# vitskvara/VBMatrixFactorization.jl

Measured on NVIDIA B200. Metric: VB iterations/s at 20000x200000x64 (dense vbmf, Float64), higher is better.
Workload: dtype f64

## Files before the change

### vbmatrixfactorization.jl_b200/csrc/capi.cu

```cuda
#include "../../include/vbmf_b200.h"
#include "common.cuh"
#include "gemm.cuh"
#include "kernels.cuh"

#include <atomic>
#include <type_traits>
#include <cstdarg>
#include <cstdlib>
#include <cstring>
#include <dlfcn.h>
#include <unistd.h>
#include <string>
#include <vector>
#include <algorithm>
#include <thread>

namespace vb {

static thread_local char g_err[1024] = "";
void set_error(const char* fmt, ...) {
    va_list ap;
    va_start(ap, fmt);
    vsnprintf(g_err, sizeof(g_err), fmt, ap);
    va_end(ap);
// ... 46 lines not shown
        }                                                                                       \
    } while (0)

}

using namespace vb;

struct vbmf_b200_ctx {
    int device = 0, rank = 0, world = 1, num_sms = 148;
    cudaStream_t st = nullptr;
    bool own_stream = false;
    void* comm = nullptr;
    double* Y = nullptr;
    size_t Y_cap = 0;
    int L_cap = 0;
    int L = 0, Mloc = 0, Mglob = 0, moff = 0, ldY = 0;
    double* rowY2 = nullptr;
    double* d_tr = nullptr;
    double* stats_part = nullptr;
    double trYTY = 0.0;
    CUtensorMap tmY1, tmY2;
    bool have_Y = false;
    cudaStream_t copy_st = nullptr, stat_st = nullptr;
    std::vector<cudaEvent_t> ev_chunk;
    std::vector<int> chunk_c0, chunk_n;
    cudaEvent_t ev_stats = nullptr;
    int chunks_pending = 0;
    bool tr_pending = false;
    bool simt = false;
    bool gemm_dmma = false;
    uint8_t* Z = nullptr;
    int* Zexp = nullptr;
    size_t Z_bytes = 0;
    int ldZ = 0;
    bool z_ready = false, z_failed = false;
    CUtensorMap tmZ1, tmZ2;
    bool profile = false;
    std::vector<cudaEvent_t> ev_k1, ev_k2, ev_ar;
    std::vector<std::pair<int, cudaEvent_t>> ev_seg;
    struct Px {
        bool ok = false, failed = false, claimed = false;
        char* local = nullptr;
        size_t cap = 0;
        char* peer[PX_MAX_WORLD] = {};
        bool ipc[PX_MAX_WORLD] = {};
        char* xchg = nullptr;
        unsigned long long epoch = 0;
        unsigned long long* wait_ns = nullptr;
    } px;
    bool profile_segments = false;
    char* batch_dev = nullptr;
    char* batch_host = nullptr;
    size_t batch_bytes = 0;
};

static int ctx_allreduce(vbmf_b200_ctx* c, double* buf, size_t n) {
    if (c->world <= 1 || n == 0) return 0;
    VB_NCCL_OK(g_nccl.AllReduce(buf, buf, n,  8,  0, c->comm, c->st));
    return 0;
}

struct PxRec {
    long long pid;
    unsigned long long host;
    unsigned long long ptr;
    int dev, ok;
    cudaIpcMemHandle_t h;
    char pad[128 - 32 - sizeof(cudaIpcMemHandle_t)];
};
// ... 279 lines not shown
        if (ctx_allreduce(c, c->rowY2, (size_t)c->L)) return -1;
        if (k_total(c->st, c->rowY2, c->L, c->d_tr)) return -1;
    }
    VB_CUDA_OK(cudaMemcpyAsync(&c->trYTY, c->d_tr, 8, cudaMemcpyDeviceToHost, c->st));
    VB_CUDA_OK(cudaStreamSynchronize(c->st));
    c->have_Y = true;
    return 0;
}

static int ctx_wait_upload(vbmf_b200_ctx* c) {
    if (c->chunks_pending > 0) {
        VB_CUDA_OK(cudaStreamWaitEvent(c->st, c->ev_stats, 0));
        c->chunks_pending = 0;
    }
    return 0;
}
static int ctx_host_trYTY(vbmf_b200_ctx* c) {
    if (c->tr_pending) {
        VB_CUDA_OK(cudaEventSynchronize(c->ev_stats));
        VB_CUDA_OK(cudaMemcpy(&c->trYTY, c->d_tr, 8, cudaMemcpyDeviceToHost));
        c->tr_pending = false;
    }
    return 0;
}
static size_t align_up(size_t x, size_t a) { return (x + a - 1) / a * a; }

static bool ctx_int8_wanted(const vbmf_b200_ctx* c, int64_t H) {
    return !c->simt && !c->gemm_dmma && H >= 1 && H <= 64 && c->Y != nullptr && c->Mloc > 0;
}
static int ctx_slices(vbmf_b200_ctx* c, bool* ok) {
    *ok = false;
    if (c->z_failed || c->Y == nullptr || c->Mloc <= 0) return 0;
    if (c->z_ready) { *ok = true; return 0; }
    const int ldZ = i8_ld(c->L);
    const size_t bytes = (size_t)I8_NSL * c->Mloc * ldZ;
    if (c->Z == nullptr || c->Z_bytes != bytes || c->ldZ != ldZ) {
        ctx_free_Z(c);
        if (cudaMalloc(&c->Z, bytes) != cudaSuccess || cudaMalloc(&c->Zexp, 2 * ((size_t)ldZ + c->Mloc) * 4) != cudaSuccess) {
            cudaGetLastError();
            ctx_free_Z(c);
            c->z_failed = true;
            return 0;
        }
        c->Z_bytes = bytes; c->ldZ = ldZ;
    }
    int* F = c->Zexp;
    if (i8_build_Y(c->st, c->Y, c->ldY, c->L, c->Mloc, c->Z, ldZ, F, F + c->L, F + c->L + c->Mloc, F + 2 * c->L + c->Mloc)) return -1;
    const uint64_t s1 = (uint64_t)ldZ, s2 = (uint64_t)ldZ * c->Mloc;
    if (make_tmap_3d_i8(&c->tmZ1, c->Z, (uint64_t)c->L, (uint64_t)c->Mloc, I8_NSL, s1, s2, 32, 128, I8_NSL, false)) return -1;
    if (make_tmap_3d_i8(&c->tmZ2, c->Z, (uint64_t)c->L, (uint64_t)c->Mloc, I8_NSL, s1, s2, 128, 32, I8_NSL, true)) return -1;
    c->z_ready = true;
    *ok = true;
    return 0;
}
static void i8_plans(int L, int M, int H, int num_sms, int* S1, int* kbs1, int* S, int* kchunk) {
    plan_splitk_ytb(L, M, H, num_sms, S1, kbs1);
    *kbs1 = (*kbs1 + 1) & ~1;
    const int nkb = (L + 15) / 16;
    *S1 = std::max(1, (nkb + *kbs1 - 1) / *kbs1);
    plan_splitk(L, M, H, num_sms, S, kchunk);
    *kchunk = (*kchunk + 31) / 32 * 32;
    *S = std::max(1, (M + *kchunk - 1) / *kchunk);
}
struct I8Operands {
    char* mem = nullptr;
    uint8_t *Wb = nullptr, *Wa = nullptr;
    int *Gb = nullptr, *Ga = nullptr;
    int ldM = 0;
    CUtensorMap tmWb, tmWa;
    I8Operands() = default;
    I8Operands(const I8Operands&) = delete;
    I8Operands& operator=(const I8Operands&) = delete;
    ~I8Operands() { if (mem) cudaFree(mem); }
};
static int i8_operands_alloc(I8Operands* o, int L, int M, int H, int S, bool* ok) {
    *ok = false;
    const int Hp = i8_hpad(H), ldZ = i8_ld(L);
    o->ldM = i8_ld(std::max(M, 1));
    const size_t nb = align_up((size_t)I8_NSL * Hp * ldZ, 256), na = align_up((size_t)I8_NSL * Hp * o->ldM, 256);
    const size_t gb = align_up((size_t)Hp * 4, 256), ga = align_up((size_t)S * Hp * 4, 256);
    if (cudaMalloc(&o->mem, nb + na + gb + ga) != cudaSuccess) { cudaGetLastError(); o->mem = nullptr; return 0; }
    o->Wb = (uint8_t*)o->mem; o->Wa = o->Wb + nb; o->Gb = (int*)(o->Wa + na); o->Ga = (int*)((char*)o->Gb + gb);
    if (make_tmap_3d_i8(&o->tmWb, o->Wb, (uint64_t)L, (uint64_t)Hp, I8_NSL, (uint64_t)ldZ, (uint64_t)ldZ * Hp, 32, (uint32_t)Hp, I8_NSL, false)) return -1;
    if (M > 0 && make_tmap_3d_i8(&o->tmWa, o->Wa, (uint64_t)M, (uint64_t)Hp, I8_NSL, (uint64_t)o->ldM, (uint64_t)o->ldM * Hp, 32, (uint32_t)Hp, I8_NSL, false)) return -1;
    *ok = true;
    return 0;
}
static int i8_k1(vbmf_b200_ctx* c, I8Operands* o, const double* B, int ldB, int H, double* P, int S1, int kbs1, const Scalars* sc) {
    const int* F = c->Zexp;
    const int* E = c->Zexp + c->L;
    const int* Ebad = c->Zexp + 2 * c->L + c->Mloc;
    if (i8_slice_B(c->st, B, ldB, c->L, H, F, o->Wb, c->ldZ, o->Gb, sc)) return -1;
    return launch_gemm_i8(c->st, false, &c->tmZ1, &o->tmWb, P, c->Mloc, c->L, S1, kbs1 * 16, H, E, Ebad, o->Gb, 0,
                          (size_t)c->Mloc * H, (size_t)H, 1, sc, c->num_sms);
}
static int i8_k2(vbmf_b200_ctx* c, I8Operands* o, const double* A, int H, double* Qpart, int ldQ, int S, int kchunk, const Scalars* sc) {
    const int* F = c->Zexp;
    const int* E = c->Zexp + c->L;
    const int* Fbad = c->Zexp + c->L + c->Mloc;
    if (i8_slice_A(c->st, A, c->Mloc, H, E, kchunk, S, o->Wa, o->ldM, o->Ga, sc)) return -1;
    return launch_gemm_i8(c->st, true, &c->tmZ2, &o->tmWa, Qpart, c->L, c->Mloc, S, kchunk, H, F, Fbad, o->Ga, i8_hpad(H),
                          (size_t)H * ldQ, 1, (size_t)ldQ, sc, c->num_sms);
}

static int attach_Y_chunked(vbmf_b200_ctx* c, const double* Y, int64_t ldY, int64_t chunk_cols) {
    if (!c->copy_st) VB_CUDA_OK(cudaStreamCreateWithFlags(&c->copy_st, cudaStreamNonBlocking));
    if (!c->stat_st) VB_CUDA_OK(cudaStreamCreateWithFlags(&c->stat_st, cudaStreamNonBlocking));
    if (!c->ev_stats) VB_CUDA_OK(cudaEventCreateWithFlags(&c->ev_stats, cudaEventDisableTiming));
    c->chunk_c0.clear(); c->chunk_n.clear();
    for (int64_t c0 = 0; c0 < c->Mloc; c0 += chunk_cols) { c->chunk_c0.push_back((int)c0); c->chunk_n.push_back((int)std::min<int64_t>(chunk_cols, c->Mloc - c0)); }
    const size_t nch = c->chunk_c0.size();
    while (c->ev_chunk.size() < nch) { cudaEvent_t e; VB_CUDA_OK(cudaEventCreateWithFlags(&e, cudaEventDisableTiming)); c->ev_chunk.push_back(e); }
    cudaEvent_t e0;
    VB_CUDA_OK(cudaEventCreateWithFlags(&e0, cudaEventDisableTiming));
    VB_CUDA_OK(cudaEventRecord(e0, c->st));
    VB_CUDA_OK(cudaStreamWaitEvent(c->copy_st, e0, 0));
    VB_CUDA_OK(cudaStreamWaitEvent(c->stat_st, e0, 0));
    VB_CUDA_OK(cudaEventDestroy(e0));
    Dev d;
    memset(&d, 0, sizeof(d));
    d.L = c->L; d.Mloc = c->Mloc; d.Y = c->Y; d.ldY = c->ldY; d.rowY2 = c->rowY2; d.part = c->stats_part;
    for (size_t k = 0; k < nch; ++k) {
        const size_t c0 = (size_t)c->chunk_c0[k], n = (size_t)c->chunk_n[k];
        if (ldY == c->L && c->ldY == c->L)
            VB_CUDA_OK(cudaMemcpyAsync(c->Y + c0 * c->ldY, Y + c0 * (size_t)ldY, (size_t)c->L * n * 8, cudaMemcpyHostToDevice, c->copy_st));
        else
            VB_CUDA_OK(cudaMemcpy2DAsync(c->Y + c0 * c->ldY, (size_t)c->ldY * 8, Y + c0 * (size_t)ldY, (size_t)ldY * 8, (size_t)c->L * 8, n,
                                         cudaMemcpyHostToDevice, c->copy_st));
        VB_CUDA_OK(cudaEventRecord(c->ev_chunk[k], c->copy_st));
        VB_CUDA_OK(cudaStreamWaitEvent(c->stat_st, c->ev_chunk[k], 0));
        if (k_y_stats_chunk(c->stat_st, d, (int)c0, (int)n, k == 0 ? 1 : 0)) return -1;
    }
    if (c->world > 1) VB_NCCL_OK(g_nccl.AllReduce(c->rowY2, c->rowY2, (size_t)c->L, 8, 0, c->comm, c->stat_st));
    if (k_total(c->stat_st, c->rowY2, c->L, c->d_tr)) return -1;
// ... 1681 lines not shown
```

### vbmatrixfactorization.jl_b200/csrc/gemm.cuh

```cuda
#pragma once
#include "common.cuh"

namespace vb {

typedef CUresult (*PFN_encodeTiled)(CUtensorMap*, CUtensorMapDataType, cuuint32_t, void*, const cuuint64_t*,
                                    const cuuint64_t*, const cuuint32_t*, const cuuint32_t*, CUtensorMapInterleave,
                                    CUtensorMapSwizzle, CUtensorMapL2promotion, CUtensorMapFloatOOBfill);
PFN_encodeTiled tmap_encoder();

int make_tmap_2d(CUtensorMap* out, const void* base, uint64_t dim0, uint64_t dim1, uint64_t stride1_bytes,
                 uint32_t box0, uint32_t box1);

struct GemmGeometry {
    int bn;
    int ctas_per_sm;
    int stages;
};
GemmGeometry gemm_geometry(int H);
int gemm_init_device();

int launch_gemm_ytb(cudaStream_t st, const CUtensorMap* tmY, const CUtensorMap* tmB, double* P,
                    int M, int L, int H, int ldP, int S, int kb_per_split, size_t slab_stride, const Scalars* sc, int num_sms);
void plan_splitk_ytb(int L, int M, int H, int num_sms, int* S, int* kb_per_split);

int launch_gemm_ya(cudaStream_t st, const CUtensorMap* tmY, const CUtensorMap* tmA, double* Qpart,
                   int L, int M, int H, int ldQ, int kchunk, int S, const Scalars* sc, int num_sms);

void plan_splitk(int L, int M, int H, int num_sms, int* S, int* kchunk);

constexpr int I8_NSL = 7;
inline int i8_hpad(int H) { return (H + 15) / 16 * 16; }
inline int i8_ld(int n) { return (n + 15) / 16 * 16; }
int gemm_i8_init_device();
int make_tmap_3d_i8(CUtensorMap* out, const void* base, uint64_t d0, uint64_t d1, uint64_t d2, uint64_t s1, uint64_t s2,
                    uint32_t b0, uint32_t b1, uint32_t b2, bool swizzle128);
int i8_build_Y(cudaStream_t st, const double* Y, int ldY, int L, int M, uint8_t* Z, int ldZ, int* F, int* E, int* Fbad, int* Ebad);
int i8_slice_B(cudaStream_t st, const double* B, int ldB, int L, int H, const int* F, uint8_t* W, int ldZ, int* G, const Scalars* sc);
int i8_slice_A(cudaStream_t st, const double* A, int M, int H, const int* E, int kchunk, int S, uint8_t* W, int ldM, int* G, const Scalars* sc);
int launch_gemm_i8(cudaStream_t st, bool mn, const CUtensorMap* tmA, const CUtensorMap* tmB, double* out, int nrows, int kdim,
                   int S, int klen, int H, const int* rowexp, const int* rowbad, const int* colexp, int cstride, size_t slab,
                   size_t rs, size_t hs, const Scalars* sc, int num_sms);

int launch_gemm_ytb_simt(cudaStream_t st, const double* Y, int ldY, const double* B, int ldB, double* P,
                         int M, int L, int H, int ldP, const Scalars* sc);
int launch_gemm_ya_simt(cudaStream_t st, const double* Y, int ldY, const double* A, double* Qpart,
                        int L, int M, int H, int ldQ, int kchunk, int S, const Scalars* sc);

}
```

### vbmatrixfactorization.jl_b200/csrc/gemm_int8.cu

```cuda
#include "gemm.cuh"
#include <algorithm>

namespace vb {
namespace i8k {

constexpr int TM = 128;
constexpr int KB = 32;
constexpr int NSL = I8_NSL;
constexpr int STAGES = 4;
constexpr int A_BYTES = NSL * TM * KB;
constexpr int B_BYTES = NSL * 64 * KB;
constexpr int SB = A_BYTES + B_BYTES;
static_assert(SB % 1024 == 0 && A_BYTES % 1024 == 0, "stage layout must stay 1024-byte aligned");
constexpr int SMEM = STAGES * SB + 1024 + 256;
static_assert(SMEM <= 227 * 1024, "stage ring exceeds the shared memory of one CTA");
constexpr int SEG_KB = 16384 / KB;
static_assert((long long)SEG_KB * KB * NSL * 128 * 128 < (1ll << 31), "level 6 may overflow INT32 between flushes");
constexpr int EXP_NONE = -(1 << 30);
constexpr int EXP_NAN = 1 << 30;

__device__ __forceinline__ uint32_t smem_u32(const void* p) { return (uint32_t)__cvta_generic_to_shared(p); }
__device__ __forceinline__ void mbar_init(uint32_t bar, uint32_t count) {
    asm volatile("mbarrier.init.shared::cta.b64 [%0], %1;" ::"r"(bar), "r"(count) : "memory");
}
__device__ __forceinline__ void mbar_expect_tx(uint32_t bar, uint32_t bytes) {
    asm volatile("mbarrier.arrive.expect_tx.shared::cta.b64 _, [%0], %1;" ::"r"(bar), "r"(bytes) : "memory");
}
__device__ __forceinline__ void mbar_arrive(uint32_t bar) {
    asm volatile("mbarrier.arrive.shared::cta.b64 _, [%0];" ::"r"(bar) : "memory");
}
__device__ __forceinline__ void mbar_wait(uint32_t bar, uint32_t parity) {
    uint32_t ok;
    do {
        asm volatile(
            "{\n\t.reg .pred p;\n\t"
            "mbarrier.try_wait.parity.shared::cta.b64 p, [%1], %2;\n\t"
            "selp.u32 %0, 1, 0, p;\n\t}"
            : "=r"(ok) : "r"(bar), "r"(parity) : "memory");
    } while (!ok);
}
__device__ __forceinline__ void tma_load_3d(uint32_t dst, const CUtensorMap* tm, uint32_t bar, int c0, int c1, int c2) {
    asm volatile(
        "cp.async.bulk.tensor.3d.shared::cluster.global.mbarrier::complete_tx::bytes [%0], [%1, {%3, %4, %5}], [%2];"
        ::"r"(dst), "l"(tm), "r"(bar), "r"(c0), "r"(c1), "r"(c2) : "memory");
}
__device__ __forceinline__ void tc_fence_before() { asm volatile("tcgen05.fence::before_thread_sync;" ::: "memory"); }
__device__ __forceinline__ void tc_fence_after() { asm volatile("tcgen05.fence::after_thread_sync;" ::: "memory"); }
__device__ __forceinline__ void tc_commit(uint32_t bar) {
    asm volatile("tcgen05.commit.cta_group::1.mbarrier::arrive::one.shared::cluster.b64 [%0];" ::"r"(bar) : "memory");
}
__device__ __forceinline__ void mma_i8(uint32_t d, uint64_t a, uint64_t b, uint32_t idesc, uint32_t acc) {
    asm volatile(
        "{\n\t.reg .pred p;\n\tsetp.ne.b32 p, %4, 0;\n\t"
        "tcgen05.mma.cta_group::1.kind::i8 [%0], %1, %2, %3, p;\n\t}"
        ::"r"(d), "l"(a), "l"(b), "r"(idesc), "r"(acc) : "memory");
}
__device__ __forceinline__ void tmem_ld8(uint32_t taddr, uint32_t (&v)[8]) {
    asm volatile("tcgen05.ld.sync.aligned.32x32b.x8.b32 {%0,%1,%2,%3,%4,%5,%6,%7}, [%8];"
                 : "=r"(v[0]), "=r"(v[1]), "=r"(v[2]), "=r"(v[3]), "=r"(v[4]), "=r"(v[5]), "=r"(v[6]), "=r"(v[7])
                 : "r"(taddr) : "memory");
}
__device__ __forceinline__ void tmem_wait_ld() { asm volatile("tcgen05.wait::ld.sync.aligned;" ::: "memory"); }

__device__ __forceinline__ uint64_t sdesc(uint32_t addr, uint32_t lbo, uint32_t sbo, uint32_t layout) {
    return (uint64_t)((addr & 0x3FFFFu) >> 4) | ((uint64_t)(lbo >> 4) << 16) | ((uint64_t)(sbo >> 4) << 32) | (1ull << 46) |
           ((uint64_t)layout << 61);
}
constexpr uint32_t LAYOUT_SW128 = 2, LAYOUT_SW32 = 6;

__device__ __forceinline__ int exp_of(double x) {
    if (x == 0.0 || !isfinite(x)) return EXP_NONE;
    int e;
    frexp(x, &e);
    return e;
}
__device__ __forceinline__ int exp_digits(double x) {
    if (x == 0.0 || !isfinite(x)) return EXP_NONE;
    int e;
    const double m = frexp(x, &e);
    return fabs(m) > 127.0 / 128.0 ? e + 1 : e;
}
__device__ __forceinline__ int exp_fix(int e) { return e <= EXP_NONE ? 0 : e; }

__device__ __forceinline__ long long fixed55(double x, int e) { return isfinite(x) ? __double2ll_rn(ldexp(x, 55 - e)) : 0ll; }

__device__ __forceinline__ void digits4(const long long (&x)[4], uint32_t (&out)[NSL]) {
#pragma unroll
    for (int i = 0; i < NSL; ++i) out[i] = 0u;
#pragma unroll
    for (int q = 0; q < 4; ++q) {
        long long t = x[q];
#pragma unroll
        for (int i = NSL - 1; i >= 0; --i) {
            const int d = (int8_t)(t & 255);
            out[i] |= ((uint32_t)t & 0xffu) << (8 * q);
            t = (t - d) >> 8;
        }
    }
}

__device__ __forceinline__ int block_max_int(int v, int* red) {
#pragma unroll
    for (int o = 16; o > 0; o >>= 1) v = max(v, __shfl_xor_sync(0xffffffffu, v, o));
    const int w = threadIdx.x >> 5, l = threadIdx.x & 31;
    __syncthreads();
    if (l == 0) red[w] = v;
    __syncthreads();
    if (w == 0) {
        v = l < (int)(blockDim.x >> 5) ? red[l] : EXP_NONE;
#pragma unroll
        for (int o = 16; o > 0; o >>= 1) v = max(v, __shfl_xor_sync(0xffffffffu, v, o));
        if (l == 0) red[0] = v;
    }
    __syncthreads();
    return red[0];
}

__global__ void __launch_bounds__(256) y_row_exp_kernel(const double* __restrict__ Y, int ldY, int L, int M, int* __restrict__ F,
                                                        int* __restrict__ Fbad) {
    const int l = blockIdx.x * blockDim.x + threadIdx.x;
    if (l >= L) return;
    int e = EXP_NONE;
    bool bad = false;
    for (int m = blockIdx.y; m < M; m += gridDim.y) {
        const double y = Y[(size_t)m * ldY + l];
        e = max(e, exp_of(y));
        bad |= !isfinite(y);
    }
    atomicMax(F + l, e);
    if (bad) Fbad[l] = 1;
}

__global__ void __launch_bounds__(256) y_slices_kernel(const double* __restrict__ Y, int ldY, int L, int M, const int* __restrict__ F,
                                                       int* __restrict__ E, int* __restrict__ Ebad, uint8_t* __restrict__ Z, int ldZ) {
    __shared__ int red[32];
    const int m = blockIdx.x;
    const double* y = Y + (size_t)m * ldY;
    int e = EXP_NONE, bad = 0;
    for (int l = threadIdx.x; l < L; l += blockDim.x) {
        const int ey = exp_digits(y[l]);
        if (ey > EXP_NONE) e = max(e, ey - exp_fix(F[l]));
        bad |= !isfinite(y[l]);
    }
    bad = __syncthreads_or(bad);
    const int Em = exp_fix(block_max_int(e, red));
    if (threadIdx.x == 0) { E[m] = Em; Ebad[m] = bad; }
    const size_t plane = (size_t)M * ldZ;
    for (int l4 = threadIdx.x; l4 < ldZ / 4; l4 += blockDim.x) {
        long long x[4];
#pragma unroll
        for (int q = 0; q < 4; ++q) {
            const int l = 4 * l4 + q;
            x[q] = l < L ? fixed55(y[l], exp_fix(F[l]) + Em) : 0;
        }
        uint32_t s[NSL];
        digits4(x, s);
#pragma unroll
        for (int i = 0; i < NSL; ++i) reinterpret_cast<uint32_t*>(Z + i * plane + (size_t)m * ldZ)[l4] = s[i];
    }
}

__global__ void __launch_bounds__(512) b_slices_kernel(const double* __restrict__ B, int ldB, int L, int H, int Hp, const int* __restrict__ F,
                                                       uint8_t* __restrict__ W, int ldZ, int* __restrict__ G, const Scalars* __restrict__ sc) {
    if (sc != nullptr && !sc->active) return;
    __shared__ int red[32];
    const int h = blockIdx.x;
    const double* b = B + (size_t)h * ldB;
    int e = EXP_NONE, bad = 0;
    if (h < H)
        for (int l = threadIdx.x; l < L; l += blockDim.x) {
            const int eb = exp_digits(b[l]);
            if (eb > EXP_NONE) e = max(e, eb + exp_fix(F[l]));
            bad |= !isfinite(b[l]);
        }
    bad = __syncthreads_or(bad);
    const int Gh = bad ? EXP_NAN : exp_fix(block_max_int(e, red));
    if (threadIdx.x == 0) G[h] = Gh;
    const size_t plane = (size_t)Hp * ldZ;
    for (int l4 = threadIdx.x; l4 < ldZ / 4; l4 += blockDim.x) {
        long long x[4];
#pragma unroll
        for (int q = 0; q < 4; ++q) {
            const int l = 4 * l4 + q;
            x[q] = (h < H && l < L) ? fixed55(b[l], Gh - exp_fix(F[l])) : 0;
        }
        uint32_t s[NSL];
        digits4(x, s);
#pragma unroll
        for (int i = 0; i < NSL; ++i) reinterpret_cast<uint32_t*>(W + i * plane + (size_t)h * ldZ)[l4] = s[i];
    }
}

__global__ void __launch_bounds__(256) a_exp_kernel(const double* __restrict__ A, int M, int H, int Hp, const int* __restrict__ E, int kchunk,
                                                    int* __restrict__ G, const Scalars* __restrict__ sc) {
    if (sc != nullptr && !sc->active) return;
    const int h = threadIdx.x & 63;
    if (h >= H) return;
    const int m0 = blockIdx.x * 256, m1 = min(M, m0 + 256);
    int cur = -1, e = EXP_NONE;
    for (int m = m0 + (threadIdx.x >> 6); m < m1; m += 4) {
        const int c = m / kchunk;
        if (c != cur) {
            if (cur >= 0 && e > EXP_NONE) atomicMax(G + cur * Hp + h, e);
            cur = c; e = EXP_NONE;
        }
        const double a = A[(size_t)m * H + h];
        const int ea = exp_digits(a);
        if (!isfinite(a)) e = EXP_NAN;
        else if (ea > EXP_NONE) e = max(e, ea + E[m]);
    }
    if (cur >= 0 && e > EXP_NONE) atomicMax(G + cur * Hp + h, e);
}

__global__ void __launch_bounds__(256) a_slices_kernel(const double* __restrict__ A, int M, int H, int Hp, const int* __restrict__ E, int kchunk,
                                                       const int* __restrict__ G, uint8_t* __restrict__ W, int ldM, const Scalars* __restrict__ sc) {
    if (sc != nullptr && !sc->active) return;
    __shared__ double tile[64 * 64];
    const int m0 = blockIdx.x * 64;
    const int nm = min(64, M - m0);
    for (int t = threadIdx.x; t < nm * H; t += blockDim.x) tile[t] = A[(size_t)m0 * H + t];
    __syncthreads();
    const size_t plane = (size_t)Hp * ldM;
    for (int t = threadIdx.x; t < Hp * 16; t += blockDim.x) {
        const int h = t >> 4, g = t & 15;
        if (m0 + 4 * g >= ldM) continue;
        long long x[4];
#pragma unroll
        for (int q = 0; q < 4; ++q) {
            const int r = 4 * g + q, m = m0 + r;
            x[q] = 0;
            if (h < H && r < nm) x[q] = fixed55(tile[r * H + h], exp_fix(G[(m / kchunk) * Hp + h]) - E[m]);
        }
        uint32_t s[NSL];
        digits4(x, s);
#pragma unroll
        for (int i = 0; i < NSL; ++i) reinterpret_cast<uint32_t*>(W + i * plane + (size_t)h * ldM + m0)[g] = s[i];
    }
}

template <bool MN>
__global__ void __launch_bounds__(192, 1)
gemm_i8_kernel(const __grid_constant__ CUtensorMap tmA, const __grid_constant__ CUtensorMap tmB, double* __restrict__ out,
               int nrows, int kdim, int S, int klen, int H, int Hp, const int* __restrict__ rowexp,
               const int* __restrict__ rowbad, const int* __restrict__ colexp, int cstride, size_t slab, size_t rs, size_t hs, const Scalars* __restrict__ sc) {
    if (sc != nullptr && !sc->active) return;
    extern __shared__ uint8_t smem_raw[];
    const uint32_t base = (smem_u32(smem_raw) + 1023u) & ~1023u;
    const uint32_t full0 = base + STAGES * SB, empty0 = full0 + STAGES * 8;
    const uint32_t tfull = empty0 + STAGES * 8, tempty = tfull + 8, tslot = tempty + 8;
    uint32_t* tslot_ptr = reinterpret_cast<uint32_t*>(smem_raw + (tslot - smem_u32(smem_raw)));

    const int warp = threadIdx.x >> 5, lane = threadIdx.x & 31;
    const uint32_t ncols = Hp * NSL <= 128 ? 128 : (Hp * NSL <= 256 ? 256 : 512);
    if (threadIdx.x == 0) {
        for (int s = 0; s < STAGES; ++s) { mbar_init(full0 + 8 * s, 1); mbar_init(empty0 + 8 * s, 1); }
        mbar_init(tfull, 1);
        mbar_init(tempty, 4);
        asm volatile("fence.mbarrier_init.release.cluster;" ::: "memory");
        asm volatile("fence.proxy.async.shared::cta;" ::: "memory");
    }
    if (warp == 5) {
        asm volatile("tcgen05.alloc.cta_group::1.sync.aligned.shared::cta.b32 [%0], %1;" ::"r"(tslot), "r"(ncols) : "memory");
        asm volatile("tcgen05.relinquish_alloc_permit.cta_group::1.sync.aligned;" ::: "memory");
    }
    tc_fence_before();
    __syncthreads();
    tc_fence_after();
    const uint32_t tmem = *reinterpret_cast<volatile uint32_t*>(tslot_ptr);

    const int ntile = (nrows + TM - 1) / TM;
    const int nwork = ntile * S;
    const uint32_t tx_bytes = A_BYTES + NSL * Hp * KB;

    if (warp == 4) {
        if (lane == 0) {
            uint32_t it = 0;
            for (int w = blockIdx.x; w < nwork; w += gridDim.x) {
                const int r0 = (w % ntile) * TM, k0 = (w / ntile) * klen, k1 = min(kdim, k0 + klen);
                for (int k = k0; k < k1; k += KB, ++it) {
                    const uint32_t s = it % STAGES, ph = (it / STAGES) & 1;
                    mbar_wait(empty0 + 8 * s, ph ^ 1);
                    mbar_expect_tx(full0 + 8 * s, tx_bytes);
                    if (MN) tma_load_3d(base + s * SB, &tmA, full0 + 8 * s, r0, k, 0);
                    else tma_load_3d(base + s * SB, &tmA, full0 + 8 * s, k, r0, 0);
                    tma_load_3d(base + s * SB + A_BYTES, &tmB, full0 + 8 * s, k, 0, 0);
                }
            }
        }
    } else if (warp == 5) {
        if (lane == 0) {
            const uint32_t idesc0 = (2u << 4) | (1u << 7) | (1u << 10) | ((MN ? 1u : 0u) << 15) | ((uint32_t)(TM >> 4) << 24);
            uint32_t it = 0, sg = 0;
            for (int w = blockIdx.x; w < nwork; w += gridDim.x) {
                const int k0 = (w / ntile) * klen, k1 = min(kdim, k0 + klen);
                const int nkb = (k1 - k0 + KB - 1) / KB;
                for (int kb0 = 0; kb0 < nkb; kb0 += SEG_KB, ++sg) {
                    const int kb1 = min(nkb, kb0 + SEG_KB);
                    mbar_wait(tempty, (sg & 1) ^ 1);
                    tc_fence_after();
                    for (int kb = kb0; kb < kb1; ++kb, ++it) {
                        const uint32_t s = it % STAGES, ph = (it / STAGES) & 1;
                        mbar_wait(full0 + 8 * s, ph);
                        tc_fence_after();
                        const uint32_t a0 = base + s * SB, b0 = a0 + A_BYTES;
#pragma unroll
                        for (int i = 0; i < NSL; ++i) {
                            const uint64_t ad = MN ? sdesc(a0 + i * (TM * KB), 16, 1024, LAYOUT_SW128)
                                                   : sdesc(a0 + i * (TM * KB), 16, 256, LAYOUT_SW32);
                            const int ntot = Hp * (NSL - i);
                            for (int p = 0; p < ntot; p += 256) {
                                const int n = min(256, ntot - p);
                                const uint64_t bd = sdesc(b0 + p * KB, 16, 256, LAYOUT_SW32);
                                mma_i8(tmem + Hp * i + p, ad, bd, idesc0 | ((uint32_t)(n >> 3) << 17), (kb > kb0 || i > 0) ? 1u : 0u);
                            }
                        }
                        tc_commit(empty0 + 8 * s);
                    }
                    tc_commit(tfull);
                }
            }
        }
    } else {
        const uint32_t lane_base = (uint32_t)(warp * 32) << 16;
        uint32_t sg = 0;
        for (int w = blockIdx.x; w < nwork; w += gridDim.x) {
            const int tile = w % ntile, sp = w / ntile;
            const int k0 = sp * klen, k1 = min(kdim, k0 + klen);
            const int nkb = (k1 - k0 + KB - 1) / KB;
            const int row = tile * TM + warp * 32 + lane;
            const bool live = row < nrows;
            const int re = live ? rowexp[row] : 0;
            const bool bad = live && rowbad[row] != 0;
            double* o = out + (size_t)sp * slab + (size_t)(live ? row : 0) * rs;
            const int* ce = colexp + (size_t)sp * cstride;
            for (int kb0 = 0; kb0 < nkb; kb0 += SEG_KB, ++sg) {
                mbar_wait(tfull, sg & 1);
                tc_fence_after();
                for (int h0 = 0; h0 < Hp; h0 += 8) {
                    uint32_t v[NSL][8];
#pragma unroll
                    for (int k = 0; k < NSL; ++k) tmem_ld8(tmem + lane_base + Hp * k + h0, v[k]);
                    tmem_wait_ld();
#pragma unroll
                    for (int c = 0; c < 8; ++c) {
                        const int h = h0 + c;
                        double acc = (double)(int)v[NSL - 1][c];
#pragma unroll
                        for (int k = NSL - 2; k >= 0; --k) acc = fma(acc, 0x1p-8, (double)(int)v[k][c]);
                        if (live && h < H) {
                            const double x = (bad || ce[h] == EXP_NAN) ? __longlong_as_double(0x7ff8000000000000ll)
                                                                       : ldexp(acc, re + ce[h] - 14);
                            double* p = o + (size_t)h * hs;
                            *p = kb0 == 0 ? x : *p + x;
                        }
                    }
                }
                tc_fence_before();
                __syncwarp();
                if (lane == 0) mbar_arrive(tempty);
            }
        }
    }
    tc_fence_before();
    __syncthreads();
    if (warp == 5) {
        tc_fence_after();
        asm volatile("tcgen05.dealloc.cta_group::1.sync.aligned.b32 %0, %1;" ::"r"(tmem), "r"(ncols) : "memory");
    }
}

}
using namespace i8k;

int make_tmap_3d_i8(CUtensorMap* out, const void* base, uint64_t d0, uint64_t d1, uint64_t d2, uint64_t s1, uint64_t s2,
                    uint32_t b0, uint32_t b1, uint32_t b2, bool swizzle128) {
    PFN_encodeTiled enc = tmap_encoder();
    if (!enc) return -1;
    if ((reinterpret_cast<uintptr_t>(base) & 15) != 0 || (s1 & 15) != 0 || (s2 & 15) != 0) {
        set_error("INT8 tensor map needs a 16-byte aligned base and pitches (base=%p pitches %llu, %llu)", base,
                  (unsigned long long)s1, (unsigned long long)s2);
        return -1;
    }
    cuuint64_t dims[3] = {d0, d1, d2};
    cuuint64_t strides[2] = {s1, s2};
    cuuint32_t box[3] = {b0, b1, b2};
    cuuint32_t estr[3] = {1, 1, 1};
    CUresult r = enc(out, CU_TENSOR_MAP_DATA_TYPE_UINT8, 3, const_cast<void*>(base), dims, strides, box, estr,
                     CU_TENSOR_MAP_INTERLEAVE_NONE, swizzle128 ? CU_TENSOR_MAP_SWIZZLE_128B : CU_TENSOR_MAP_SWIZZLE_32B,
                     CU_TENSOR_MAP_L2_PROMOTION_L2_128B, CU_TENSOR_MAP_FLOAT_OOB_FILL_NONE);
    if (r != CUDA_SUCCESS) {
        set_error("cuTensorMapEncodeTiled (int8) failed with CUresult %d (dims %llu x %llu x %llu, box %u x %u x %u)", (int)r,
                  (unsigned long long)d0, (unsigned long long)d1, (unsigned long long)d2, b0, b1, b2);
        return -1;
    }
    return 0;
}

int gemm_i8_init_device() {
    VB_CUDA_OK(cudaFuncSetAttribute(gemm_i8_kernel<false>, cudaFuncAttributeMaxDynamicSharedMemorySize, SMEM));
    VB_CUDA_OK(cudaFuncSetAttribute(gemm_i8_kernel<true>, cudaFuncAttributeMaxDynamicSharedMemorySize, SMEM));
    return 0;
}

int i8_build_Y(cudaStream_t st, const double* Y, int ldY, int L, int M, uint8_t* Z, int ldZ, int* F, int* E, int* Fbad, int* Ebad) {
    if (L <= 0 || M <= 0) return 0;
    VB_CUDA_OK(cudaMemsetAsync(F, 0x80, (size_t)L * 4, st));
    VB_CUDA_OK(cudaMemsetAsync(Fbad, 0, (size_t)L * 4, st));
    dim3 g1((L + 255) / 256, std::min(M, 512));
    y_row_exp_kernel<<<g1, 256, 0, st>>>(Y, ldY, L, M, F, Fbad);
    VB_LAUNCH_OK();
    y_slices_kernel<<<M, 256, 0, st>>>(Y, ldY, L, M, F, E, Ebad, Z, ldZ);
    VB_LAUNCH_OK();
    return 0;
}

int i8_slice_B(cudaStream_t st, const double* B, int ldB, int L, int H, const int* F, uint8_t* W, int ldZ, int* G, const Scalars* sc) {
    const int Hp = i8_hpad(H);
    b_slices_kernel<<<Hp, 512, 0, st>>>(B, ldB, L, H, Hp, F, W, ldZ, G, sc);
    VB_LAUNCH_OK();
    return 0;
}

int i8_slice_A(cudaStream_t st, const double* A, int M, int H, const int* E, int kchunk, int S, uint8_t* W, int ldM, int* G, const Scalars* sc) {
    if (M <= 0) return 0;
    const int Hp = i8_hpad(H);
    VB_CUDA_OK(cudaMemsetAsync(G, 0x80, (size_t)S * Hp * 4, st));
    a_exp_kernel<<<(M + 255) / 256, 256, 0, st>>>(A, M, H, Hp, E, kchunk, G, sc);
    VB_LAUNCH_OK();
    a_slices_kernel<<<(ldM + 63) / 64, 256, 0, st>>>(A, M, H, Hp, E, kchunk, G, W, ldM, sc);
    VB_LAUNCH_OK();
    return 0;
}

int launch_gemm_i8(cudaStream_t st, bool mn, const CUtensorMap* tmA, const CUtensorMap* tmB, double* out, int nrows, int kdim,
                   int S, int klen, int H, const int* rowexp, const int* rowbad, const int* colexp, int cstride, size_t slab,
                   size_t rs, size_t hs, const Scalars* sc, int num_sms) {
    if (H > 64) { set_error("H = %d > 64 is not supported by the INT8 contraction", H); return -1; }
    if (klen % KB != 0) { set_error("INT8 split-K chunk %d is not a multiple of %d", klen, KB); return -1; }
    if (nrows <= 0 || kdim <= 0 || H <= 0) return 0;
    const int nwork = ((nrows + TM - 1) / TM) * S;
    const int grid = std::max(1, std::min(nwork, num_sms));
    if (mn) gemm_i8_kernel<true><<<grid, 192, SMEM, st>>>(*tmA, *tmB, out, nrows, kdim, S, klen, H, i8_hpad(H), rowexp, rowbad, colexp, cstride, slab, rs, hs, sc);
    else gemm_i8_kernel<false><<<grid, 192, SMEM, st>>>(*tmA, *tmB, out, nrows, kdim, S, klen, H, i8_hpad(H), rowexp, rowbad, colexp, cstride, slab, rs, hs, sc);
    VB_LAUNCH_OK();
    return 0;
}

}
```

Measured before the change: 64.48.

## Store INT8 slices in pre-swizzled tile-blocked layout and load with bulk copies

Replaces the TMA tensor-map loads of the INT8 digit-sliced Y and weight operands with plain cp.async.bulk copies. The slices are now written by the slicing kernels directly in the shared-memory tile layout (32-byte swizzled, padded to 128), so each pipeline stage is a contiguous block. The non-transposed path needs one bulk copy per stage. The transposed path issues 28 smaller 1 KB copies and switches its descriptor from SW128 to SW32. This removes tensor-map setup and any TMA tiling overhead, but it adds more padding memory and more copy instructions on the transposed path.

```diff
diff --git a/vbmatrixfactorization.jl_b200/csrc/capi.cu b/vbmatrixfactorization.jl_b200/csrc/capi.cu
--- a/vbmatrixfactorization.jl_b200/csrc/capi.cu
+++ b/vbmatrixfactorization.jl_b200/csrc/capi.cu
@@ -102,9 +102,8 @@
     uint8_t* Z = nullptr;
     int* Zexp = nullptr;
     size_t Z_bytes = 0;
-    int ldZ = 0;
+    int Z_Lp = 0;
     bool z_ready = false, z_failed = false;
-    CUtensorMap tmZ1, tmZ2;
     bool profile = false;
     std::vector<cudaEvent_t> ev_k1, ev_k2, ev_ar;
     std::vector<std::pair<int, cudaEvent_t>> ev_seg;
@@ -450,23 +449,20 @@
     *ok = false;
     if (c->z_failed || c->Y == nullptr || c->Mloc <= 0) return 0;
     if (c->z_ready) { *ok = true; return 0; }
-    const int ldZ = i8_ld(c->L);
-    const size_t bytes = (size_t)I8_NSL * c->Mloc * ldZ;
-    if (c->Z == nullptr || c->Z_bytes != bytes || c->ldZ != ldZ) {
+    const int Lp = i8_pad(c->L), Mp = i8_pad(c->Mloc);
+    const size_t bytes = i8_z_bytes(c->L, c->Mloc);
+    if (c->Z == nullptr || c->Z_bytes != bytes || c->Z_Lp != Lp) {
         ctx_free_Z(c);
-        if (cudaMalloc(&c->Z, bytes) != cudaSuccess || cudaMalloc(&c->Zexp, 2 * ((size_t)ldZ + c->Mloc) * 4) != cudaSuccess) {
+        if (cudaMalloc(&c->Z, bytes) != cudaSuccess || cudaMalloc(&c->Zexp, 2 * ((size_t)Lp + Mp) * 4) != cudaSuccess) {
             cudaGetLastError();
             ctx_free_Z(c);
             c->z_failed = true;
             return 0;
         }
-        c->Z_bytes = bytes; c->ldZ = ldZ;
+        c->Z_bytes = bytes; c->Z_Lp = Lp;
     }
     int* F = c->Zexp;
-    if (i8_build_Y(c->st, c->Y, c->ldY, c->L, c->Mloc, c->Z, ldZ, F, F + c->L, F + c->L + c->Mloc, F + 2 * c->L + c->Mloc)) return -1;
-    const uint64_t s1 = (uint64_t)ldZ, s2 = (uint64_t)ldZ * c->Mloc;
-    if (make_tmap_3d_i8(&c->tmZ1, c->Z, (uint64_t)c->L, (uint64_t)c->Mloc, I8_NSL, s1, s2, 32, 128, I8_NSL, false)) return -1;
-    if (make_tmap_3d_i8(&c->tmZ2, c->Z, (uint64_t)c->L, (uint64_t)c->Mloc, I8_NSL, s1, s2, 128, 32, I8_NSL, true)) return -1;
+    if (i8_build_Y(c->st, c->Y, c->ldY, c->L, c->Mloc, c->Z, F, F + c->L, F + c->L + c->Mloc, F + 2 * c->L + c->Mloc)) return -1;
     c->z_ready = true;
     *ok = true;
     return 0;
@@ -484,8 +480,6 @@
     char* mem = nullptr;
     uint8_t *Wb = nullptr, *Wa = nullptr;
     int *Gb = nullptr, *Ga = nullptr;
-    int ldM = 0;
-    CUtensorMap tmWb, tmWa;
     I8Operands() = default;
     I8Operands(const I8Operands&) = delete;
     I8Operands& operator=(const I8Operands&) = delete;
@@ -493,14 +487,11 @@
 };
 static int i8_operands_alloc(I8Operands* o, int L, int M, int H, int S, bool* ok) {
     *ok = false;
-    const int Hp = i8_hpad(H), ldZ = i8_ld(L);
-    o->ldM = i8_ld(std::max(M, 1));
-    const size_t nb = align_up((size_t)I8_NSL * Hp * ldZ, 256), na = align_up((size_t)I8_NSL * Hp * o->ldM, 256);
+    const int Hp = i8_hpad(H);
+    const size_t nb = align_up(i8_operand_bytes(L, H), 256), na = align_up(i8_operand_bytes(M, H), 256);
     const size_t gb = align_up((size_t)Hp * 4, 256), ga = align_up((size_t)S * Hp * 4, 256);
     if (cudaMalloc(&o->mem, nb + na + gb + ga) != cudaSuccess) { cudaGetLastError(); o->mem = nullptr; return 0; }
     o->Wb = (uint8_t*)o->mem; o->Wa = o->Wb + nb; o->Gb = (int*)(o->Wa + na); o->Ga = (int*)((char*)o->Gb + gb);
-    if (make_tmap_3d_i8(&o->tmWb, o->Wb, (uint64_t)L, (uint64_t)Hp, I8_NSL, (uint64_t)ldZ, (uint64_t)ldZ * Hp, 32, (uint32_t)Hp, I8_NSL, false)) return -1;
-    if (M > 0 && make_tmap_3d_i8(&o->tmWa, o->Wa, (uint64_t)M, (uint64_t)Hp, I8_NSL, (uint64_t)o->ldM, (uint64_t)o->ldM * Hp, 32, (uint32_t)Hp, I8_NSL, false)) return -1;
     *ok = true;
     return 0;
 }
@@ -508,16 +499,16 @@
     const int* F = c->Zexp;
     const int* E = c->Zexp + c->L;
     const int* Ebad = c->Zexp + 2 * c->L + c->Mloc;
-    if (i8_slice_B(c->st, B, ldB, c->L, H, F, o->Wb, c->ldZ, o->Gb, sc)) return -1;
-    return launch_gemm_i8(c->st, false, &c->tmZ1, &o->tmWb, P, c->Mloc, c->L, S1, kbs1 * 16, H, E, Ebad, o->Gb, 0,
+    if (i8_slice_B(c->st, B, ldB, c->L, H, F, o->Wb, o->Gb, sc)) return -1;
+    return launch_gemm_i8(c->st, false, c->Z, o->Wb, P, c->Mloc, c->L, S1, kbs1 * 16, H, E, Ebad, o->Gb, 0,
                           (size_t)c->Mloc * H, (size_t)H, 1, sc, c->num_sms);
 }
 static int i8_k2(vbmf_b200_ctx* c, I8Operands* o, const double* A, int H, double* Qpart, int ldQ, int S, int kchunk, const Scalars* sc) {
     const int* F = c->Zexp;
     const int* E = c->Zexp + c->L;
     const int* Fbad = c->Zexp + c->L + c->Mloc;
-    if (i8_slice_A(c->st, A, c->Mloc, H, E, kchunk, S, o->Wa, o->ldM, o->Ga, sc)) return -1;
-    return launch_gemm_i8(c->st, true, &c->tmZ2, &o->tmWa, Qpart, c->L, c->Mloc, S, kchunk, H, F, Fbad, o->Ga, i8_hpad(H),
+    if (i8_slice_A(c->st, A, c->Mloc, H, E, kchunk, S, o->Wa, o->Ga, sc)) return -1;
+    return launch_gemm_i8(c->st, true, c->Z, o->Wa, Qpart, c->L, c->Mloc, S, kchunk, H, F, Fbad, o->Ga, i8_hpad(H),
                           (size_t)H * ldQ, 1, (size_t)ldQ, sc, c->num_sms);
 }
 
diff --git a/vbmatrixfactorization.jl_b200/csrc/gemm.cuh b/vbmatrixfactorization.jl_b200/csrc/gemm.cuh
--- a/vbmatrixfactorization.jl_b200/csrc/gemm.cuh
+++ b/vbmatrixfactorization.jl_b200/csrc/gemm.cuh
@@ -30,14 +30,14 @@
 
 constexpr int I8_NSL = 7;
 inline int i8_hpad(int H) { return (H + 15) / 16 * 16; }
-inline int i8_ld(int n) { return (n + 15) / 16 * 16; }
+__host__ __device__ inline int i8_pad(int n) { return (n + 127) / 128 * 128; }
 int gemm_i8_init_device();
-int make_tmap_3d_i8(CUtensorMap* out, const void* base, uint64_t d0, uint64_t d1, uint64_t d2, uint64_t s1, uint64_t s2,
-                    uint32_t b0, uint32_t b1, uint32_t b2, bool swizzle128);
-int i8_build_Y(cudaStream_t st, const double* Y, int ldY, int L, int M, uint8_t* Z, int ldZ, int* F, int* E, int* Fbad, int* Ebad);
-int i8_slice_B(cudaStream_t st, const double* B, int ldB, int L, int H, const int* F, uint8_t* W, int ldZ, int* G, const Scalars* sc);
-int i8_slice_A(cudaStream_t st, const double* A, int M, int H, const int* E, int kchunk, int S, uint8_t* W, int ldM, int* G, const Scalars* sc);
-int launch_gemm_i8(cudaStream_t st, bool mn, const CUtensorMap* tmA, const CUtensorMap* tmB, double* out, int nrows, int kdim,
+size_t i8_z_bytes(int L, int M);
+size_t i8_operand_bytes(int kdim, int H);
+int i8_build_Y(cudaStream_t st, const double* Y, int ldY, int L, int M, uint8_t* Z, int* F, int* E, int* Fbad, int* Ebad);
+int i8_slice_B(cudaStream_t st, const double* B, int ldB, int L, int H, const int* F, uint8_t* W, int* G, const Scalars* sc);
+int i8_slice_A(cudaStream_t st, const double* A, int M, int H, const int* E, int kchunk, int S, uint8_t* W, int* G, const Scalars* sc);
+int launch_gemm_i8(cudaStream_t st, bool mn, const uint8_t* Z, const uint8_t* W, double* out, int nrows, int kdim,
                    int S, int klen, int H, const int* rowexp, const int* rowbad, const int* colexp, int cstride, size_t slab,
                    size_t rs, size_t hs, const Scalars* sc, int num_sms);
 
diff --git a/vbmatrixfactorization.jl_b200/csrc/gemm_int8.cu b/vbmatrixfactorization.jl_b200/csrc/gemm_int8.cu
--- a/vbmatrixfactorization.jl_b200/csrc/gemm_int8.cu
+++ b/vbmatrixfactorization.jl_b200/csrc/gemm_int8.cu
@@ -39,10 +39,9 @@
             : "=r"(ok) : "r"(bar), "r"(parity) : "memory");
     } while (!ok);
 }
-__device__ __forceinline__ void tma_load_3d(uint32_t dst, const CUtensorMap* tm, uint32_t bar, int c0, int c1, int c2) {
-    asm volatile(
-        "cp.async.bulk.tensor.3d.shared::cluster.global.mbarrier::complete_tx::bytes [%0], [%1, {%3, %4, %5}], [%2];"
-        ::"r"(dst), "l"(tm), "r"(bar), "r"(c0), "r"(c1), "r"(c2) : "memory");
+__device__ __forceinline__ void bulk_load(uint32_t dst, const void* src, uint32_t bytes, uint32_t bar) {
+    asm volatile("cp.async.bulk.shared::cluster.global.mbarrier::complete_tx::bytes [%0], [%1], %2, [%3];"
+                 ::"r"(dst), "l"(src), "r"(bytes), "r"(bar) : "memory");
 }
 __device__ __forceinline__ void tc_fence_before() { asm volatile("tcgen05.fence::before_thread_sync;" ::: "memory"); }
 __device__ __forceinline__ void tc_fence_after() { asm volatile("tcgen05.fence::after_thread_sync;" ::: "memory"); }
@@ -66,7 +65,7 @@
     return (uint64_t)((addr & 0x3FFFFu) >> 4) | ((uint64_t)(lbo >> 4) << 16) | ((uint64_t)(sbo >> 4) << 32) | (1ull << 46) |
            ((uint64_t)layout << 61);
 }
-constexpr uint32_t LAYOUT_SW128 = 2, LAYOUT_SW32 = 6;
+constexpr uint32_t LAYOUT_SW32 = 6;
 
 __device__ __forceinline__ int exp_of(double x) {
     if (x == 0.0 || !isfinite(x)) return EXP_NONE;
@@ -132,36 +131,44 @@
 }
 
 __global__ void __launch_bounds__(256) y_slices_kernel(const double* __restrict__ Y, int ldY, int L, int M, const int* __restrict__ F,
-                                                       int* __restrict__ E, int* __restrict__ Ebad, uint8_t* __restrict__ Z, int ldZ) {
+                                                       int* __restrict__ E, int* __restrict__ Ebad, uint8_t* __restrict__ Z) {
     __shared__ int red[32];
     const int m = blockIdx.x;
-    const double* y = Y + (size_t)m * ldY;
-    int e = EXP_NONE, bad = 0;
-    for (int l = threadIdx.x; l < L; l += blockDim.x) {
-        const int ey = exp_digits(y[l]);
-        if (ey > EXP_NONE) e = max(e, ey - exp_fix(F[l]));
-        bad |= !isfinite(y[l]);
-    }
-    bad = __syncthreads_or(bad);
-    const int Em = exp_fix(block_max_int(e, red));
-    if (threadIdx.x == 0) { E[m] = Em; Ebad[m] = bad; }
-    const size_t plane = (size_t)M * ldZ;
-    for (int l4 = threadIdx.x; l4 < ldZ / 4; l4 += blockDim.x) {
+    const bool live = m < M;
+    const double* y = Y + (size_t)(live ? m : 0) * ldY;
+    int Em = 0;
+    if (live) {
+        int e = EXP_NONE, bad = 0;
+        for (int l = threadIdx.x; l < L; l += blockDim.x) {
+            const int ey = exp_digits(y[l]);
+            if (ey > EXP_NONE) e = max(e, ey - exp_fix(F[l]));
+            bad |= !isfinite(y[l]);
+        }
+        bad = __syncthreads_or(bad);
+        Em = exp_fix(block_max_int(e, red));
+        if (threadIdx.x == 0) { E[m] = Em; Ebad[m] = bad; }
+    }
+    const int Lp = i8_pad(L);
+    const size_t lstride = (size_t)(i8_pad(M) / TM) * A_BYTES;
+    uint8_t* zc = Z + (size_t)(m / TM) * A_BYTES + (m / 32 % 4) * 1024 + 32 * (m % 32);
+    const int sw = (m & 4) << 2;
+    for (int l4 = threadIdx.x; l4 < Lp / 4; l4 += blockDim.x) {
         long long x[4];
 #pragma unroll
         for (int q = 0; q < 4; ++q) {
             const int l = 4 * l4 + q;
-            x[q] = l < L ? fixed55(y[l], exp_fix(F[l]) + Em) : 0;
+            x[q] = live && l < L ? fixed55(y[l], exp_fix(F[l]) + Em) : 0;
         }
         uint32_t s[NSL];
         digits4(x, s);
-#pragma unroll
-        for (int i = 0; i < NSL; ++i) reinterpret_cast<uint32_t*>(Z + i * plane + (size_t)m * ldZ)[l4] = s[i];
+        uint8_t* p = zc + (size_t)(l4 / 8) * lstride + ((4 * l4 % 32) ^ sw);
+#pragma unroll
+        for (int i = 0; i < NSL; ++i) *reinterpret_cast<uint32_t*>(p + i * (TM * KB)) = s[i];
     }
 }
 
 __global__ void __launch_bounds__(512) b_slices_kernel(const double* __restrict__ B, int ldB, int L, int H, int Hp, const int* __restrict__ F,
-                                                       uint8_t* __restrict__ W, int ldZ, int* __restrict__ G, const Scalars* __restrict__ sc) {
+                                                       uint8_t* __restrict__ W, int* __restrict__ G, const Scalars* __restrict__ sc) {
     if (sc != nullptr && !sc->active) return;
     __shared__ int red[32];
     const int h = blockIdx.x;
@@ -176,8 +183,8 @@
     bad = __syncthreads_or(bad);
     const int Gh = bad ? EXP_NAN : exp_fix(block_max_int(e, red));
     if (threadIdx.x == 0) G[h] = Gh;
-    const size_t plane = (size_t)Hp * ldZ;
-    for (int l4 = threadIdx.x; l4 < ldZ / 4; l4 += blockDim.x) {
+    const int Lp = i8_pad(L), sw = (h & 4) << 2;
+    for (int l4 = threadIdx.x; l4 < Lp / 4; l4 += blockDim.x) {
         long long x[4];
 #pragma unroll
         for (int q = 0; q < 4; ++q) {
@@ -186,8 +193,9 @@
         }
         uint32_t s[NSL];
         digits4(x, s);
-#pragma unroll
-        for (int i = 0; i < NSL; ++i) reinterpret_cast<uint32_t*>(W + i * plane + (size_t)h * ldZ)[l4] = s[i];
+        uint8_t* p = W + (size_t)(l4 / 8) * (NSL * Hp * KB) + h * KB + ((4 * l4 % 32) ^ sw);
+#pragma unroll
+        for (int i = 0; i < NSL; ++i) *reinterpret_cast<uint32_t*>(p + i * Hp * KB) = s[i];
     }
 }
 
@@ -213,17 +221,15 @@
 }
 
 __global__ void __launch_bounds__(256) a_slices_kernel(const double* __restrict__ A, int M, int H, int Hp, const int* __restrict__ E, int kchunk,
-                                                       const int* __restrict__ G, uint8_t* __restrict__ W, int ldM, const Scalars* __restrict__ sc) {
+                                                       const int* __restrict__ G, uint8_t* __restrict__ W, const Scalars* __restrict__ sc) {
     if (sc != nullptr && !sc->active) return;
     __shared__ double tile[64 * 64];
     const int m0 = blockIdx.x * 64;
-    const int nm = min(64, M - m0);
+    const int nm = max(0, min(64, M - m0));
     for (int t = threadIdx.x; t < nm * H; t += blockDim.x) tile[t] = A[(size_t)m0 * H + t];
     __syncthreads();
-    const size_t plane = (size_t)Hp * ldM;
     for (int t = threadIdx.x; t < Hp * 16; t += blockDim.x) {
         const int h = t >> 4, g = t & 15;
-        if (m0 + 4 * g >= ldM) continue;
         long long x[4];
 #pragma unroll
         for (int q = 0; q < 4; ++q) {
@@ -233,14 +239,16 @@
         }
         uint32_t s[NSL];
         digits4(x, s);
-#pragma unroll
-        for (int i = 0; i < NSL; ++i) reinterpret_cast<uint32_t*>(W + i * plane + (size_t)h * ldM + m0)[g] = s[i];
+        const int mw = m0 + 4 * g;
+        uint8_t* p = W + (size_t)(mw / 32) * (NSL * Hp * KB) + h * KB + ((mw % 32) ^ ((h & 4) << 2));
+#pragma unroll
+        for (int i = 0; i < NSL; ++i) *reinterpret_cast<uint32_t*>(p + i * Hp * KB) = s[i];
     }
 }
 
 template <bool MN>
 __global__ void __launch_bounds__(192, 1)
-gemm_i8_kernel(const __grid_constant__ CUtensorMap tmA, const __grid_constant__ CUtensorMap tmB, double* __restrict__ out,
+gemm_i8_kernel(const uint8_t* __restrict__ Z, const uint8_t* __restrict__ W, double* __restrict__ out,
                int nrows, int kdim, int S, int klen, int H, int Hp, const int* __restrict__ rowexp,
                const int* __restrict__ rowbad, const int* __restrict__ colexp, int cstride, size_t slab, size_t rs, size_t hs, const Scalars* __restrict__ sc) {
     if (sc != nullptr && !sc->active) return;
@@ -270,20 +278,29 @@
 
     const int ntile = (nrows + TM - 1) / TM;
     const int nwork = ntile * S;
-    const uint32_t tx_bytes = A_BYTES + NSL * Hp * KB;
-
+    const uint32_t wstage = NSL * Hp * KB;
+    const uint32_t tx_bytes = A_BYTES + wstage;
+
+    const size_t nmb = i8_pad(MN ? kdim : nrows) / TM;
     if (warp == 4) {
         if (lane == 0) {
             uint32_t it = 0;
             for (int w = blockIdx.x; w < nwork; w += gridDim.x) {
                 const int r0 = (w % ntile) * TM, k0 = (w / ntile) * klen, k1 = min(kdim, k0 + klen);
                 for (int k = k0; k < k1; k += KB, ++it) {
-                    const uint32_t s = it % STAGES, ph = (it / STAGES) & 1;
+                    const uint32_t s = it % STAGES, ph = (it / STAGES) & 1, bar = full0 + 8 * s, a0 = base + s * SB;
                     mbar_wait(empty0 + 8 * s, ph ^ 1);
-                    mbar_expect_tx(full0 + 8 * s, tx_bytes);
-                    if (MN) tma_load_3d(base + s * SB, &tmA, full0 + 8 * s, r0, k, 0);
-                    else tma_load_3d(base + s * SB, &tmA, full0 + 8 * s, k, r0, 0);
-                    tma_load_3d(base + s * SB + A_BYTES, &tmB, full0 + 8 * s, k, 0, 0);
+                    mbar_expect_tx(bar, tx_bytes);
+                    if (MN) {
+                        const uint8_t* z = Z + ((size_t)(r0 / 32) * nmb + k / TM) * A_BYTES + (k / 32 % 4) * 1024;
+#pragma unroll 1
+                        for (int j = 0; j < 4; ++j, z += (size_t)nmb * A_BYTES)
+#pragma unroll
+                            for (int i = 0; i < NSL; ++i) bulk_load(a0 + i * (TM * KB) + j * 1024, z + i * (TM * KB), 1024, bar);
+                    } else {
+                        bulk_load(a0, Z + ((size_t)(k / 32) * nmb + r0 / TM) * A_BYTES, A_BYTES, bar);
+                    }
+                    bulk_load(a0 + A_BYTES, W + (size_t)(k / 32) * wstage, wstage, bar);
                 }
             }
         }
@@ -305,7 +322,7 @@
                         const uint32_t a0 = base + s * SB, b0 = a0 + A_BYTES;
 #pragma unroll
                         for (int i = 0; i < NSL; ++i) {
-                            const uint64_t ad = MN ? sdesc(a0 + i * (TM * KB), 16, 1024, LAYOUT_SW128)
+                            const uint64_t ad = MN ? sdesc(a0 + i * (TM * KB), 1024, 256, LAYOUT_SW32)
                                                    : sdesc(a0 + i * (TM * KB), 16, 256, LAYOUT_SW32);
                             const int ntot = Hp * (NSL - i);
                             for (int p = 0; p < ntot; p += 256) {
@@ -372,29 +389,8 @@
 }
 using namespace i8k;
 
-int make_tmap_3d_i8(CUtensorMap* out, const void* base, uint64_t d0, uint64_t d1, uint64_t d2, uint64_t s1, uint64_t s2,
-                    uint32_t b0, uint32_t b1, uint32_t b2, bool swizzle128) {
-    PFN_encodeTiled enc = tmap_encoder();
-    if (!enc) return -1;
-    if ((reinterpret_cast<uintptr_t>(base) & 15) != 0 || (s1 & 15) != 0 || (s2 & 15) != 0) {
-        set_error("INT8 tensor map needs a 16-byte aligned base and pitches (base=%p pitches %llu, %llu)", base,
-                  (unsigned long long)s1, (unsigned long long)s2);
-        return -1;
-    }
-    cuuint64_t dims[3] = {d0, d1, d2};
-    cuuint64_t strides[2] = {s1, s2};
-    cuuint32_t box[3] = {b0, b1, b2};
-    cuuint32_t estr[3] = {1, 1, 1};
-    CUresult r = enc(out, CU_TENSOR_MAP_DATA_TYPE_UINT8, 3, const_cast<void*>(base), dims, strides, box, estr,
-                     CU_TENSOR_MAP_INTERLEAVE_NONE, swizzle128 ? CU_TENSOR_MAP_SWIZZLE_128B : CU_TENSOR_MAP_SWIZZLE_32B,
-                     CU_TENSOR_MAP_L2_PROMOTION_L2_128B, CU_TENSOR_MAP_FLOAT_OOB_FILL_NONE);
-    if (r != CUDA_SUCCESS) {
-        set_error("cuTensorMapEncodeTiled (int8) failed with CUresult %d (dims %llu x %llu x %llu, box %u x %u x %u)", (int)r,
-                  (unsigned long long)d0, (unsigned long long)d1, (unsigned long long)d2, b0, b1, b2);
-        return -1;
-    }
-    return 0;
-}
+size_t i8_z_bytes(int L, int M) { return (size_t)NSL * i8_pad(L) * i8_pad(M); }
+size_t i8_operand_bytes(int kdim, int H) { return (size_t)NSL * i8_hpad(H) * i8_pad(kdim); }
 
 int gemm_i8_init_device() {
     VB_CUDA_OK(cudaFuncSetAttribute(gemm_i8_kernel<false>, cudaFuncAttributeMaxDynamicSharedMemorySize, SMEM));
@@ -402,37 +398,37 @@
     return 0;
 }
 
-int i8_build_Y(cudaStream_t st, const double* Y, int ldY, int L, int M, uint8_t* Z, int ldZ, int* F, int* E, int* Fbad, int* Ebad) {
+int i8_build_Y(cudaStream_t st, const double* Y, int ldY, int L, int M, uint8_t* Z, int* F, int* E, int* Fbad, int* Ebad) {
     if (L <= 0 || M <= 0) return 0;
     VB_CUDA_OK(cudaMemsetAsync(F, 0x80, (size_t)L * 4, st));
     VB_CUDA_OK(cudaMemsetAsync(Fbad, 0, (size_t)L * 4, st));
     dim3 g1((L + 255) / 256, std::min(M, 512));
     y_row_exp_kernel<<<g1, 256, 0, st>>>(Y, ldY, L, M, F, Fbad);
     VB_LAUNCH_OK();
-    y_slices_kernel<<<M, 256, 0, st>>>(Y, ldY, L, M, F, E, Ebad, Z, ldZ);
+    y_slices_kernel<<<i8_pad(M), 256, 0, st>>>(Y, ldY, L, M, F, E, Ebad, Z);
     VB_LAUNCH_OK();
     return 0;
 }
 
-int i8_slice_B(cudaStream_t st, const double* B, int ldB, int L, int H, const int* F, uint8_t* W, int ldZ, int* G, const Scalars* sc) {
+int i8_slice_B(cudaStream_t st, const double* B, int ldB, int L, int H, const int* F, uint8_t* W, int* G, const Scalars* sc) {
     const int Hp = i8_hpad(H);
-    b_slices_kernel<<<Hp, 512, 0, st>>>(B, ldB, L, H, Hp, F, W, ldZ, G, sc);
+    b_slices_kernel<<<Hp, 512, 0, st>>>(B, ldB, L, H, Hp, F, W, G, sc);
     VB_LAUNCH_OK();
     return 0;
 }
 
-int i8_slice_A(cudaStream_t st, const double* A, int M, int H, const int* E, int kchunk, int S, uint8_t* W, int ldM, int* G, const Scalars* sc) {
+int i8_slice_A(cudaStream_t st, const double* A, int M, int H, const int* E, int kchunk, int S, uint8_t* W, int* G, const Scalars* sc) {
     if (M <= 0) return 0;
     const int Hp = i8_hpad(H);
     VB_CUDA_OK(cudaMemsetAsync(G, 0x80, (size_t)S * Hp * 4, st));
     a_exp_kernel<<<(M + 255) / 256, 256, 0, st>>>(A, M, H, Hp, E, kchunk, G, sc);
     VB_LAUNCH_OK();
-    a_slices_kernel<<<(ldM + 63) / 64, 256, 0, st>>>(A, M, H, Hp, E, kchunk, G, W, ldM, sc);
+    a_slices_kernel<<<i8_pad(M) / 64, 256, 0, st>>>(A, M, H, Hp, E, kchunk, G, W, sc);
     VB_LAUNCH_OK();
     return 0;
 }
 
-int launch_gemm_i8(cudaStream_t st, bool mn, const CUtensorMap* tmA, const CUtensorMap* tmB, double* out, int nrows, int kdim,
+int launch_gemm_i8(cudaStream_t st, bool mn, const uint8_t* Z, const uint8_t* W, double* out, int nrows, int kdim,
                    int S, int klen, int H, const int* rowexp, const int* rowbad, const int* colexp, int cstride, size_t slab,
                    size_t rs, size_t hs, const Scalars* sc, int num_sms) {
     if (H > 64) { set_error("H = %d > 64 is not supported by the INT8 contraction", H); return -1; }
@@ -440,8 +436,8 @@
     if (nrows <= 0 || kdim <= 0 || H <= 0) return 0;
     const int nwork = ((nrows + TM - 1) / TM) * S;
     const int grid = std::max(1, std::min(nwork, num_sms));
-    if (mn) gemm_i8_kernel<true><<<grid, 192, SMEM, st>>>(*tmA, *tmB, out, nrows, kdim, S, klen, H, i8_hpad(H), rowexp, rowbad, colexp, cstride, slab, rs, hs, sc);
-    else gemm_i8_kernel<false><<<grid, 192, SMEM, st>>>(*tmA, *tmB, out, nrows, kdim, S, klen, H, i8_hpad(H), rowexp, rowbad, colexp, cstride, slab, rs, hs, sc);
+    if (mn) gemm_i8_kernel<true><<<grid, 192, SMEM, st>>>(Z, W, out, nrows, kdim, S, klen, H, i8_hpad(H), rowexp, rowbad, colexp, cstride, slab, rs, hs, sc);
+    else gemm_i8_kernel<false><<<grid, 192, SMEM, st>>>(Z, W, out, nrows, kdim, S, klen, H, i8_hpad(H), rowexp, rowbad, colexp, cstride, slab, rs, hs, sc);
     VB_LAUNCH_OK();
     return 0;
 }
```

Result: faster. 65.59 (median of 6 runs) (+1.7%).
